# Slienteagle-wyb/tdmpc

Hardware: AMD Instinct MI355X
Metric: plan-steps/sec (N=512, H=5, iters=6) at 1/2/4/8 MI355X vs CPU ref (higher is better)
Workload: dtype fp32

## Files before the change

tdmpc_amd/csrc/tdmpc_kernels.hip:

```cpp
#include <hip/hip_runtime.h>
#include <hiprand/hiprand_kernel.h>

#include <math.h>
#include <stdint.h>
#include <stdio.h>
#include <stdlib.h>
#include <string.h>
#include <unistd.h>

#include <algorithm>
#include <atomic>
#include <chrono>
#include <mutex>
#include <type_traits>
#include <vector>

#include "../../include/tdmpc_hip.h"

typedef float floatx16 __attribute__((ext_vector_type(16)));

#define DEVI __device__ __forceinline__

#ifdef TDMPC_STAMPS
__device__ unsigned long long* g_stamps;
// ... 164 lines not shown
        w->fold_w = take((size_t)2 * w->M * w->M);
        int r, k;
        x6_shape(*w, X6_WP1, &r, &k);
        w->fpi_x6 = take(rup(r, 32) * rup(k, 16) * 3 / 2);
        w->fpi_b = take((size_t)w->M);
        x6_shape(*w, X6_WQ1X, &r, &k);
        w->fq_x6 = take(rup(r, 32) * rup(k, 16) * 3 / 2);
        w->fq_b = take((size_t)2 * w->M);
        w->fold_p = take((size_t)w->M * w->M);
        w->fold_q = take((size_t)2 * w->M * w->M);
        x6_shape(*w, X6_W1X, &r, &k);
        w->fw1_x6 = take(rup(r, 32) * rup(k, 16) * 3 / 2);
    }
    w->total = o;
    return true;
}

constexpr int SPLIT_S = 4;
constexpr int SPLIT_MAX_ROWS = 4096;

struct Work {
    float* X;
    float* H1;
    float* H2;
    float2* st1;
    float2* st2;
    float* rpart;
    float* G;
    float* rlast;
    float* value;
    float* qv;
    float* z0c;
    float* pimu;
    float* zpart;
    float* rpart_s;
    int split_rows;
    float* z0;
    float* mean;
    float* stdv;
    float* enc_tmp;
    size_t x_stride;
    int xrows;
    char* p1;
    size_t p1_bytes;
    size_t total;
};

size_t pixel_act_floats(const Layout& w) {
    size_t m = 0;
    for (int i = 1; i <= 4; ++i) m = std::max(m, (size_t)w.nch * w.conv_hw[i] * w.conv_hw[i]);
    return m;
}

constexpr int P1_NG = 8;
constexpr int P1_WPG = 32;
constexpr int P1_RTM = 3;
constexpr int P1_ROWS = 32 * P1_RTM;
constexpr int P1_H1LD = 544;
constexpr unsigned P1_XCC_TAB = P1_NG * 256 + 256;
constexpr unsigned P1_SPIN_MAX = 400000;

struct P1Region {
    unsigned o_sync, o_xb, o_h1, o_zp, o_rp, o_pp, o_qm, o_qp, o_val, o_rl, o_mu, o_y2, xb_t, xb_g, total;
};

inline int p1_ks(const Layout& w) { return (w.Kx + 31) / 32 <= 4 ? 4 : 6; }
// ... 31 lines not shown
    const size_t HA = (size_t)H * A;
    return ((size_t)32 * 3 * 64 * 4 + (size_t)P1_ROWS * 36 + 2 * P1_ROWS + p1_cem_floats(H, K, A, T) +
            3 * rup(HA, 4) + 64 + 64 + 16 + 32 + 648) * 4;
}

inline bool p1_dims_ok(const tdmpc_dims* d, const Layout& w) {
    if (w.M != 512 || d->num_elites > 64) return false;
    const int N = d->num_samples, P = d->num_pi, T = N + P;
    const int sr = (N + P1_NG - 1) / P1_NG, pr = (P + P1_NG - 1) / P1_NG;
    if (sr + pr > P1_ROWS || T > 1024) return false;
    if ((w.Kx + 15) / 16 > 12 || (w.Lp + 15) / 16 > 12 || w.Lr > 128 || w.Ar > 128) return false;
    return p1_lds_bytes(d->max_horizon, d->num_elites, w.A, T) <= 160 * 1024;
}

void make_work(const tdmpc_dims* d, const Layout& w, char* base, Work* k, int extra = 0) {
    const size_t B = d->max_batch, N = d->num_samples, P = d->num_pi, T = N + P + extra, H = d->max_horizon;
    const size_t M = w.M;
    size_t o = 0;
    auto take = [&](size_t bytes) { size_t r = o; o += rup(bytes, 256); return base ? base + r : nullptr; };
    k->xrows = (int)rup(B * T, 32);
    k->x_stride = (size_t)k->xrows * w.Kx;
    k->X = (float*)take((H + 1) * k->x_stride * 4);
    k->H1 = (float*)take((size_t)k->xrows * 2 * M * 4);
    k->H2 = (float*)take((size_t)k->xrows * 2 * M * 4);
    k->st1 = (float2*)take(B * T * (2 * M / 64) * 8);
    k->st2 = (float2*)take(B * T * (2 * M / 64) * 8);
    k->rpart = (float*)take(B * T * (M / 32) * 4);
    k->G = (float*)take(B * T * 4);
    k->rlast = (float*)take(B * T * 4);
    k->value = (float*)take(B * T * 4);
    k->qv = (float*)take(2 * (size_t)k->xrows * 4);
    k->pimu = (float*)take((size_t)k->xrows * w.Ap * 4);
    k->z0c = (float*)take(B * 2 * M * 4);
    k->split_rows = std::min(k->xrows, SPLIT_MAX_ROWS);
    k->zpart = (float*)take((size_t)2 * SPLIT_S * k->split_rows * std::max(w.Lr, w.Ar) * 4);
    k->rpart_s = (float*)take((size_t)2 * SPLIT_S * k->split_rows * 4);
    k->z0 = (float*)take(B * w.Lp * 4);
    k->mean = (float*)take(B * H * w.A * 4);
    k->stdv = (float*)take(B * H * w.A * 4);
    k->enc_tmp = (float*)take(d->modality ? 2 * B * pixel_act_floats(w) * 4 : 256);
    k->p1_bytes = p1_dims_ok(d, w) && !extra ? p1_region(d, w).total : 0;
    k->p1 = k->p1_bytes ? (char*)take(k->p1_bytes) : nullptr;
    k->total = o;
}

size_t cem_lds_bytes(int T, int H, int K, int A) {
    const size_t nl = (T + 63) / 64;
    return nl * 64 * 8 + ((size_t)H * K * A + 64 + 4 * rup((size_t)H * A, 4) + 64 + 32) * 4;
}

bool check_dims(const tdmpc_dims* d) {
    if (!d) return false;
    if (d->num_samples <= 0 || d->num_pi < 0 || d->num_elites <= 0 || d->max_horizon <= 0 ||
        d->max_horizon > 16 || d->max_iterations <= 0 || d->max_batch <= 0) return false;
    const int T = d->num_samples + d->num_pi;
    if (d->num_elites > T || d->num_elites > 64 || T > 4096) return false;
    Layout w;
    if (!make_layout(d, &w)) return false;
    if (w.Kx > 1024 || w.M > 1024 || w.L > 1024 || w.A > 256 || w.E > 1024) return false;
    if (cem_lds_bytes(T, d->max_horizon, d->num_elites, w.A) > 160 * 1024) return false;
    return true;
}

DEVI float elu1(float x) { return x > 0.f ? x : expm1f(x); }
DEVI float fmul(float a, float b) { return __fmul_rn(a, b); }
DEVI float fadd(float a, float b) { return __fadd_rn(a, b); }
// ... 2514 lines not shown
    X(1, 1, 1, 1, 1, 32, false) X(1, 1, 1, 1, 1, 64, false) X(1, 1, 1, 1, 1, 128, false)              \
    X(1, 2, 1, 1, 1, 32, false) X(1, 2, 1, 1, 1, 64, false) X(1, 2, 1, 1, 1, 128, false)              \
    X(2, 2, 2, 2, 1, 1, true)

#define LDS_FOR_EACH(X) X(2, 1, 2, 4, 32) X(3, 1, 2, 4, 32) X(1, 1, 2, 2, 32)
#define CHAIN_FOR_EACH(X)                                                                            \
    X(CH_STEP, 1, 8, 4, 8, 0) X(CH_STEP, 2, 8, 4, 8, 0) X(CH_STEP, 4, 8, 4, 8, 0)                     \
    X(CH_PI, 1, 8, 4, 8, 0) X(CH_PI, 2, 8, 4, 8, 0) X(CH_PI, 4, 8, 4, 8, 0)                           \
    X(CH_Q, 1, 8, 4, 8, 0) X(CH_Q, 2, 8, 4, 8, 0) X(CH_Q, 4, 8, 4, 8, 0)                              \
    X(CH_STEP, 2, 8, 2, X6_D3, 1) X(CH_STEP, 4, 4, 2, 2, 1) X(CH_PI, 2, 8, 2, X6_D3, 1)               \
    X(CH_PI, 4, 4, 2, 2, 1) X(CH_Q, 2, 8, 2, X6_D3, 1) X(CH_Q, 4, 4, 2, 2, 1)
#define CHAIN16_FOR_EACH(X)                                                                          \
    X(CH_STEP, 2, 4, 4, 0) X(CH_STEP, 4, 4, 4, 0) X(CH_PI, 2, 4, 4, 0) X(CH_PI, 4, 4, 4, 0)           \
    X(CH_Q, 2, 4, 4, 0) X(CH_Q, 4, 4, 4, 0)                                                           \
    X(CH_STEP, 4, 4, 4, 1) X(CH_PI, 4, 4, 4, 1) X(CH_Q, 4, 4, 4, 1)
#define SPLIT_FOR_EACH(X) X(4, 4, 1) X(4, 4, 0)
#define CONV_TILE_FOR_EACH(X) X(1) X(2) X(4)
#define PLAN1_FOR_EACH(X) X(4) X(6)

int init_attrs() {
    static int done = 0;
    if (done) return 0;
    int rc = 0;
#define LINEAR_ATTR(...) rc |= set_max_lds<linear_kernel<__VA_ARGS__>>();
    FOR_EACH_LINEAR(LINEAR_ATTR)
#undef LINEAR_ATTR
    rc |= set_max_lds<cem_kernel>();
#define PLAN1_ATTR(KS) rc |= set_max_lds<plan1_kernel<KS>>();
    PLAN1_FOR_EACH(PLAN1_ATTR)
#undef PLAN1_ATTR
#define WIDE_ATTR(...) rc |= set_max_lds<wide_step_kernel<__VA_ARGS__>>();
    WIDE_FOR_EACH(WIDE_ATTR)
#undef WIDE_ATTR
#define WIDE_HEADS_ATTR(...) rc |= set_max_lds<wide_heads_kernel<__VA_ARGS__>>();
    WIDE_HEADS_FOR_EACH(WIDE_HEADS_ATTR)
#undef WIDE_HEADS_ATTR
    rc |= set_max_lds<qstat_chol_kernel>();
#define CONV_ATTR(PX) rc |= set_max_lds<conv_tile_kernel<PX>>();
    CONV_TILE_FOR_EACH(CONV_ATTR)
#undef CONV_ATTR
#define LDS_ATTR(...) rc |= set_max_lds<linear_lds_kernel<__VA_ARGS__, true>>() | set_max_lds<linear_lds_kernel<__VA_ARGS__, false>>();
    LDS_FOR_EACH(LDS_ATTR)
#undef LDS_ATTR
#define CHAIN_ATTR(...) rc |= set_max_lds<chain_kernel<__VA_ARGS__>>();
    CHAIN_FOR_EACH(CHAIN_ATTR)
#undef CHAIN_ATTR
#define CHAIN16_ATTR(...) rc |= set_max_lds<chain16_kernel<__VA_ARGS__>>();
    CHAIN16_FOR_EACH(CHAIN16_ATTR)
#undef CHAIN16_ATTR
    if (rc) return TDMPC_E_HIP;
    done = 1;
    return 0;
}

struct Profiler {
    int armed = 0, cfg = 0, pro = -1, n = 0, cap = 0, kdim = 0, rows = 0;
    hipEvent_t* ev = nullptr;
    double flops = 0.0;
    char kernel[128] = "";
};
thread_local Profiler g_prof;

bool prof_armed() { return g_prof.armed && g_prof.n + 2 <= g_prof.cap; }
hipError_t prof_begin(bool on, hipStream_t s) { return on ? hipEventRecord(g_prof.ev[g_prof.n], s) : hipSuccess; }
hipError_t prof_end(bool on, hipStream_t s, double flops) {
    if (!on) return hipSuccess;
    Profiler& pf = g_prof;
// ... 705 lines not shown
            p.X1 = (const unsigned short*)(c.pw + w.fq_x6) + q * x6_w1_rows_stride(c);
            p.b1 = c.pw + w.fq_b + q * M;
        }
    }
    a.q = qo ? qo : c.k.qv; a.q_ld = qo ? q_ld : c.k.xrows;
    return launch_chain(CH_Q, a, 2, c.s);
}

int wh_g1p(const Ctx& c) { return (int)rup(c.w.Lp, 32) / 32; }
int wh_nb3p(const Ctx& c) { return (int)rup(c.w.A, 16) / 16; }
int wh_g1q(const Ctx& c) { return (int)rup(c.Kx, 32) / 32; }
bool wh_instance(const Ctx& c) {
    const int g1p = wh_g1p(c), nb3 = wh_nb3p(c), g1q = wh_g1q(c), nst = c.w.nsr / 16;
#define WH_HAS(G1P, NB3P, G1Q, NSTQ) if (g1p == G1P && nb3 == NB3P && g1q == G1Q && nst == NSTQ) return true;
    WIDE_HEADS_FOR_EACH(WH_HAS)
#undef WH_HAS
    return false;
}
bool use_wide_heads(const Ctx& c) {
    static const int en = [] { const char* e = getenv("TDMPC_WIDE_HEADS"); return e ? atoi(e) : 1; }();
    if (!en || !c.w.nqs || c.w.M != 512 || !use_x6(c) || !num_cus()) return false;
    if (c.path != TDMPC_PATH_AUTO && c.path != TDMPC_PATH_CHAIN && c.path != TDMPC_PATH_WIDE) return false;
    if (c.N + c.P != c.T || c.N % 16 || c.P % 16) return false;
    if (!use_wide(c, c.B * c.N, RowMap{c.N, c.T, 0}, false) || !wh_instance(c)) return false;
    return c.P == 0 || use_chain(c, c.B * c.P, 1, CK_PI);
}
WHJob wh_job(int role, int head, int x0, int nx, int rows, RowMap map) {
    WHJob j;
    memset(&j, 0, sizeof j);
    j.role = role; j.head = head; j.x0 = x0; j.nx = nx; j.rows = rows; j.nrb = (rows + 127) / 128; j.map = map;
    j.eps_G = 1;
    return j;
}
int launch_wide_heads(const Ctx& c, const WHJob* jobs, int nj, const float* eps, float min_std) {
    const Layout& w = c.w;
    const int M = c.M;
    WHArgs a;
    memset(&a, 0, sizeof a);
    for (int i = 0; i < nj; ++i) a.job[i] = jobs[i];
    a.njob = nj;
    a.X = Xt(c, c.H); a.x_ts = (long)c.Kx * 32;
    auto q6 = [&](int i) { return (const unsigned short*)(c.pw + w.x6q[i]); };
    a.P1 = q6(X6_WP1); a.P2 = q6(X6_WP2); a.P3 = q6(X6_WP3);
    a.pb1 = c.pw + w.bp1; a.pb2 = c.pw + w.bp2; a.pb3 = c.pw + w.bp3;
    a.A = w.A; a.Ap = w.Ap; a.pq1 = w.Ap / 4; a.pkq = w.Lp / 4; a.pg1s = wh_g1p(c);
    a.eps = eps; a.min_std = min_std; a.lo = (float)(-1.0 + 1e-6); a.hi = (float)(1.0 - 1e-6);
    const int g1q = wh_g1q(c);
    for (int h = 0; h < 2; ++h) {
        WHQHead& q = a.q[h];
        q.S = (const unsigned short*)(c.pw + w.x6qs) + (size_t)h * (w.nsr / 16) * g1q * 1536;
        q.X1 = (const unsigned short*)(c.pw + w.x6qf) + (size_t)h * (M / 16) * g1q * 1536;
        q.X2 = q6(X6_WQ2) + (size_t)h * (M / 16) * (M / 32) * 1536;
        q.bs = c.pw + w.bqs + (size_t)h * w.nsr;
        q.b1 = c.pw + w.bqf + h * M; q.g1 = c.pw + w.g1 + h * M; q.be1 = c.pw + w.be1 + h * M;
        q.b2 = c.pw + w.bq2 + h * M; q.g2 = c.pw + w.g2 + h * M; q.be2 = c.pw + w.be2 + h * M;
        q.w3 = c.pw + w.wq3 + h * M; q.b3 = c.pw + w.bq3 + h;
    }
    a.qkq = c.Kx / 4; a.qg1s = g1q;
    a.qv = c.k.qv; a.q_ld = c.k.xrows;
    int slots = 0;
    bool allq = true;
    double flops = 0.0;
    for (int i = 0; i < nj; ++i) {
        const WHJob& J = jobs[i];
        if (J.rows % 16 || J.x0 < 0 || J.nx <= 0 || J.x0 + J.nx > 8) {
            snprintf(g_err, sizeof g_err, "wide heads: bad job %d", i);
            return TDMPC_E_DIMS;
        }
        slots = std::max(slots, (J.nrb + J.nx - 1) / J.nx);
        allq = allq && J.role == WH_Q;
        flops += 2.0 * J.rows * (J.role == WH_PI ? (double)w.L * M + (double)M * M + (double)M * w.A
                                                 : (double)(w.L + w.A) * M + (double)M * M + M);
    }
    if (!slots) return 0;
    const dim3 grid((unsigned)slots * 8), block(64 * WS_NW);
    const int g1p = wh_g1p(c), nb3 = wh_nb3p(c), nst = w.nsr / 16;
    Profiler& pf = g_prof;
    const bool prof = prof_armed() && pf.cfg == 4 + (allq ? CH_Q : CH_PI) && (pf.rows == 0 || jobs[0].rows == pf.rows);
    if (prof)
        snprintf(pf.kernel, sizeof pf.kernel, "wide_heads_kernel<%d, %d, %d, %d> (%s)", g1p, nb3, g1q, nst,
                 allq ? "Q1 + Q2" : "pi + Q1 + Q2 of the policy rows");
    HIPCHK(prof_begin(prof, c.s));
    bool done = false;
#define WH_LAUNCH(G1P, NB3P, G1Q, NSTQ) \
    if (!done && g1p == G1P && nb3 == NB3P && g1q == G1Q && nst == NSTQ) { \
        hipLaunchKernelGGL((wide_heads_kernel<G1P, NB3P, G1Q, NSTQ>), grid, block, \
                           ws_lds<(G1P > G1Q ? G1P : G1Q)>(), c.s, a); \
        done = true; \
    }
    WIDE_HEADS_FOR_EACH(WH_LAUNCH)
#undef WH_LAUNCH
    if (!done) { snprintf(g_err, sizeof g_err, "wide heads: no instance"); return TDMPC_E_DIMS; }
    HIPCHK(hipGetLastError());
    HIPCHK(prof_end(prof, c.s, flops));
    return 0;
}

int terminal_wide(const Ctx& c, const float* noise, long toff, float min_std) {
    const RowMap rm = {c.N, c.T, 0}, pm = {c.P, c.T, c.N};
    WHJob ja[3];
    int na = 0;
    ja[na] = wh_job(WH_PI, 0, 0, c.P > 0 ? 4 : 8, c.B * c.N, rm);
    ja[na].eps_env = c.eps_env; ja[na].eps_off = toff; ja[na].eps_G = c.N;
    ++na;
    if (c.P > 0) {
        ja[na++] = wh_job(WH_Q, 0, 4, 2, c.B * c.P, pm);
        ja[na++] = wh_job(WH_Q, 1, 6, 2, c.B * c.P, pm);
    }
    int rc;
    if ((rc = launch_wide_heads(c, ja, na, noise, min_std))) return rc;
    const WHJob jb[2] = {wh_job(WH_Q, 0, 0, 4, c.B * c.N, rm), wh_job(WH_Q, 1, 4, 4, c.B * c.N, rm)};
    return launch_wide_heads(c, jb, 2, noise, min_std);
}

int terminal_q_rows(const Ctx& c, int rows, RowMap map, float discH, bool chain) {
    const Layout& w = c.w;
    const int M = c.M;
    int rc;
    if (chain) return q_chain(c, rows, map);
    {
        LinArgs a = args0();
        a.M = rows; a.K = c.Kx; a.a_mapped = 1; a.amap = map;
        LinProb& p = a.p[0];
        p.A = xop(c, c.H, 0); p.W = wop(c, w.wq1x, c.Kx); p.bias = c.pw + w.bq1x;
        p.C = hout(c.k.H1, c, 0); p.N = p.nvalid = p.nstore = 2 * M; p.epi = EPI_LNSTATS;
        p.st_out = c.k.st1; p.st_ld = 2 * M / 64;
        if ((rc = launch_lin(a, 1, 2 * M, 1, PRO_PLAIN, c.s))) return rc;
    }
    {
        LnArgs l;
        l.Y = c.k.H1; l.O = c.k.H2; l.ts = (long)2 * M * 32; l.st = c.k.st1; l.st_ld = 2 * M / 64; l.M_ = M;
        l.rows = rows; l.g = c.pw + w.g1; l.b = c.pw + w.be1;
        hipLaunchKernelGGL(ln_tanh_kernel, dim3((rows + 31) / 32, 2), dim3(512), 0, c.s, l);
        HIPCHK(hipGetLastError());
    }
    {
        LinArgs a = args0();
        a.M = rows; a.K = M;
        for (int q = 0; q < 2; ++q) {
            LinProb& p = a.p[q];
            p.A = hop(c.k.H2, c, q * M / 4); p.W = wop(c, w.wq2 + (size_t)q * M * M, M);
            p.bias = c.pw + w.bq2 + q * M; p.C = hout(c.k.H1, c, q * M / 4); p.N = p.nvalid = p.nstore = M;
            p.epi = EPI_LNSTATS; p.st_out = c.k.st2 + q * (M / 64); p.st_ld = 2 * M / 64;
// ... 467 lines not shown
        }
    }

    const RowMap all = {T, T, 0};
    const RowMap pm = {P, T, N};
    const RowMap rm = {N, T, 0};
    if (P > 0) {
        for (int t = 0; t < H; ++t) {
            if ((rc = policy(c, t, B * P, pm, noise, c.eps_env, P, (long)t * P * c.A, prm->min_std, nullptr,
                             c.fold_policy && t >= 1)))
                return rc;
            if ((rc = step_next(c, t, B * T, all, prm->discount_pow[t], t == 0, t == H - 1)))
                return rc;
        }
    }
    CemArgs ca = cem_args0(c);
    ca.I = I;
    ca.eps = noise; ca.eps_env = c.eps_env; ca.eps_cem_off = c.eps_cem_off; ca.eps_iter = c.eps_iter;
    ca.eps_act_off = c.eps_act_off; ca.u = u; ca.prev_mean = prev_mean;
    ca.eval_mode = prm->eval_mode; ca.temperature = prm->temperature; ca.momentum = prm->momentum;
    ca.omm = prm->one_minus_momentum; ca.std_floor = prm->std_floor; ca.action = action; ca.metrics = metrics;
    ca.std_floor_p = prm->std_floor_dev;
    ca.elite_out = elite_out; ca.score_out = score_out; ca.mean_out = mean_out; ca.std_out = std_out;
    ca.value_out = value_out;
    ca.status = prm->status;
    const bool wide_heads = use_wide_heads(c);
    if (wide_heads || c.fold_heads || use_chain(c, B * T, 2, CK_Q)) {
        ca.G = c.k.G; ca.qv = c.k.qv; ca.q_ld = c.k.xrows; ca.discH = prm->discount_pow[H];
    }
    const size_t cem_lds = cem_lds_bytes(T, H, ca.K, c.A);

    const bool pi_cache = pi_cache_on() && P > 0 && use_chain(c, B * T, 1, CK_PI);
    const RowMap pmH = {P, T, N};
    for (int i = 0; i < I; ++i) {
        const long toff = c.eps_cem_off + (long)i * c.eps_iter + c.eps_term_off;
        const bool pm_in_prep = wide_heads && P > 0 && i > 0;
        if (i > 0) {
            const PiMuArgs pm = pimu_args(c, B * P, pmH, noise, c.eps_env, P, toff + (long)N * c.A, prm->min_std);
            if ((rc = prep(c, noise, i, nullptr, pm_in_prep ? &pm : nullptr))) return rc;
        }
        if (i > 0 || P == 0)
            for (int t = 0; t < H; ++t)
                if ((rc = step_next(c, t, B * N, rm, prm->discount_pow[t], t == 0, t == H - 1, 1)))
                    return rc;
        if (wide_heads) {
            if (P > 0) {
                if (i == 0) rc = policy(c, H, B * P, pmH, noise, c.eps_env, P, toff + (long)N * c.A, prm->min_std, c.k.pimu);
                if (rc || (rc = flush_split(c))) return rc;
            }
            if ((rc = terminal_wide(c, noise, toff, prm->min_std))) return rc;
        } else if (c.fold_heads) {
            if ((rc = policy(c, H, B * N, rm, noise, c.eps_env, N, toff, prm->min_std, nullptr, true))) return rc;
            if (P > 0) {
                if (i == 0 || !pi_cache)
                    rc = policy(c, H, B * P, pmH, noise, c.eps_env, P, toff + (long)N * c.A, prm->min_std,
                                pi_cache ? c.k.pimu : nullptr, c.fold_policy != 0);
                else
                    rc = policy_from_mu(c, B * P, pmH, noise, c.eps_env, P, toff + (long)N * c.A, prm->min_std);
                if (rc) return rc;
            }
            if ((rc = q_chain(c, B * N, rm, nullptr, nullptr, 0, true))) return rc;
            if (P > 0 && (rc = q_chain(c, B * P, pmH, nullptr, nullptr, 0, c.fold_policy != 0))) return rc;
        } else if (pi_cache && i > 0) {
            if ((rc = policy(c, H, B * N, rm, noise, c.eps_env, N, toff, prm->min_std))) return rc;
            if ((rc = flush_split(c))) return rc;
            if ((rc = policy_from_mu(c, B * P, pmH, noise, c.eps_env, P, toff + (long)N * c.A, prm->min_std)))
                return rc;
        } else if ((rc = policy(c, H, B * T, all, noise, c.eps_env, T, toff, prm->min_std,
                                pi_cache ? c.k.pimu : nullptr))) {
            return rc;
        }
        if (!wide_heads && !c.fold_heads && (rc = terminal_q(c, prm->discount_pow[H]))) return rc;
        ca.final_iter = i == I - 1;
        ca.iter = i;
        hipLaunchKernelGGL(cem_kernel, dim3(B), dim3(1024), cem_lds, c.s, ca);
        HIPCHK(hipGetLastError());
    }
    return 0;
}

int tdmpc_icem_sizes_for(const tdmpc_dims* d, tdmpc_sizes* out) {
    if (!d || !out) return TDMPC_E_NULL;
    if (!check_dims(d)) return TDMPC_E_DIMS;
// ... 225 lines not shown
```

tdmpc_amd/csrc/wide_heads.inc:

```

enum { WH_PI = 0, WH_Q = 1 };

#if (defined(WH_DIAG_ELU) || defined(WH_DIAG_NOSTATS) || defined(WH_DIAG_NOLN2)) && !defined(TDMPC_VARIANT)
#error "WH_DIAG_* diagnostics produce wrong results: build them only as a named variant (tdmpc_amd.build --variant)"
#endif
#ifdef WH_DIAG_NOSTATS
constexpr int WH_STATS_ON = 0;
#else
constexpr int WH_STATS_ON = 1;
#endif

struct WHJob {
    int role, head;
    int x0, nx;
    int rows, nrb;
    RowMap map;
    long eps_env, eps_off;
    int eps_G;
};

struct WHQHead {
    const unsigned short* S;
    const unsigned short* X1;
    const unsigned short* X2;
    const float* bs;
    const float *b1, *g1, *be1, *b2, *g2, *be2, *w3, *b3;
};

struct WHArgs {
    WHJob job[3]; int njob;
    float* X; long x_ts;
    const unsigned short *P1, *P2, *P3;
    const float *pb1, *pb2, *pb3;
    int A, Ap, pq1, pkq, pg1s;
    const float* eps; float min_std, lo, hi;
    WHQHead q[2];
    int qkq, qg1s;
    float* qv; long q_ld;
};

template <int G> constexpr size_t wh_lds() { return ws_lds<G>(); }

DEVI float wh_u(float x) { return __builtin_bit_cast(float, __builtin_amdgcn_readfirstlane(__builtin_bit_cast(int, x))); }
DEVI const w2cf* wh_cp(const float* p) {
    const unsigned long long u = (unsigned long long)p;
    const unsigned lo = __builtin_amdgcn_readfirstlane((unsigned)u), hi = __builtin_amdgcn_readfirstlane((unsigned)(u >> 32));
    return (const w2cf*)(((unsigned long long)hi << 32) | lo);
}

template <int G1, int NB3, int GX>
DEVI void wh_pi(const WHArgs& a, const WHJob& J, int rb, char* wsm) {
    constexpr int NS = ws_ns<GX>();
    constexpr int VM = 3 * (NS - 3);
    constexpr int SPC2 = G1 + 16;
    static_assert(NS >= 3 && NS - 1 < SPC2, "ring depth");
    const int tid = threadIdx.x, lane = tid & 63, n = lane & 15, q = lane >> 4;
    const int wave = __builtin_amdgcn_readfirstlane(tid >> 6);
    char* ring = wsm;
    p1f4* sx = (p1f4*)(wsm + NS * WS_SLOT) + wave * (G1 * 2 * 64) + lane;
    const float* sb2 = (const float*)(wsm + NS * WS_SLOT);
    const float* sb3 = sb2 + 512;
    const int m0 = rb * 128 + wave * 16;
    const bool live = m0 < J.rows;
    const int xr0 = live ? map_row(J.map, m0) : 0;
    const unsigned ring_lds = (unsigned)(size_t)(__attribute__((address_space(3))) char*)ring;
    const unsigned voff = lane * 16;
    auto src_main2 = [&](int sc, int j) __attribute__((always_inline)) -> const unsigned short* {
        if (j < G1) return a.P1 + ((size_t)(8 * sc + wave) * a.pg1s + j) * 1536;
        const int s2 = j - G1, co = s2 >> 3, st = s2 & 7;
        return a.P2 + ((size_t)(8 * (st & 3) + wave) * 16 + 2 * (2 * sc + co) + (st >> 2)) * 1536;
    };
// ... 144 lines not shown
        }
    }
    asm volatile("s_waitcnt vmcnt(0)" ::: "memory");
    if (live) {
        const int m = m0 + n_ep, xr = xr0 + n_ep;
        const float* ep = a.eps + (size_t)(m / J.eps_G) * J.eps_env + J.eps_off + (size_t)(m % J.eps_G) * a.A;
        float* xo = a.X + (size_t)(xr >> 5) * a.x_ts + (xr & 31) * 4;
#pragma unroll
        for (int jj = 0; jj < NB3; ++jj) {
            const int cq = 4 * jj + q_ep, col = 4 * cq;
            if (col < a.Ap) {
                const float4 bv = *(const float4*)(sb3 + col);
                const float o4[4] = {a3[jj][0] + bv.x, a3[jj][1] + bv.y, a3[jj][2] + bv.z, a3[jj][3] + bv.w};
                float o[4];
#pragma unroll
                for (int e = 0; e < 4; ++e) {
                    float x = 0.f;
                    if (col + e < a.A) {
                        const float muv = tanhf(o4[e]);
                        x = muv;
                        if (a.min_std > 0.f) {
                            const float ee = tclamp(fmul(ep[col + e], a.min_std), -0.3f, 0.3f);
                            x = tclamp(fadd(muv, ee), a.lo, a.hi);
                        }
                    }
                    o[e] = x;
                }
                *(float4*)(xo + (size_t)cq * 128) = make_float4(o[0], o[1], o[2], o[3]);
            }
        }
    }
}

template <int G1, int NST, int GX>
DEVI void wh_q(const WHArgs& a, const WHJob& J, int rb, char* wsm) {
    constexpr int NS = ws_ns<GX>();
    constexpr int VM = 3 * (NS - 3);
    constexpr int SPC2 = G1 + 16;
    constexpr int NSS = WH_STATS_ON * (NST / 8) * G1;
    static_assert(NST % 8 == 0 && NS >= 3 && NS - 1 < SPC2 && NS - 1 <= NSS + SPC2, "ring depth");
    const int tid = threadIdx.x, lane = tid & 63, n = lane & 15, q = lane >> 4;
    const int wave = __builtin_amdgcn_readfirstlane(tid >> 6);
    const WHQHead Hd = J.head ? a.q[1] : a.q[0];
    char* ring = wsm;
    p1f4* sx = (p1f4*)(wsm + NS * WS_SLOT) + wave * (G1 * 2 * 64) + lane;
    const float* sv = (const float*)(wsm + NS * WS_SLOT);
    const int m0 = rb * 128 + wave * 16;
    const bool live = m0 < J.rows;
    const int xr0 = live ? map_row(J.map, m0) : 0;
    const unsigned ring_lds = (unsigned)(size_t)(__attribute__((address_space(3))) char*)ring;
    const unsigned voff = lane * 16;
    auto src_main2 = [&](int sc, int j) __attribute__((always_inline)) -> const unsigned short* {
        if (sc > 3) return Hd.X2;
        if (j < G1) return Hd.X1 + ((size_t)(8 * sc + wave) * a.qg1s + j) * 1536;
        const int s2 = j - G1, co = s2 >> 3, st = s2 & 7;
        return Hd.X2 + ((size_t)(8 * (st & 3) + wave) * 16 + 2 * (2 * sc + co) + (st >> 2)) * 1536;
    };
    auto src_abs = [&](int j) __attribute__((always_inline)) -> const unsigned short* {
        if (j < NSS) return Hd.S + ((size_t)(8 * (j / G1) + wave) * a.qg1s + j % G1) * 1536;
        return src_main2((j - NSS) / SPC2, (j - NSS) % SPC2);
    };
    auto src_next2 = [&](int sc, int j) __attribute__((always_inline)) -> const unsigned short* {
        const int jt = j + NS - 1;
        if (jt < SPC2) return src_main2(sc, jt);
        return src_main2(sc + 1, jt - SPC2);
    };
    auto issue = [&](int k, const unsigned short* src) __attribute__((always_inline)) {
        const unsigned dst = ring_lds + (unsigned)((k % NS) * WS_SLOT + wave * WS_FRAG);
#pragma unroll
        for (int p = 0; p < 3; ++p) w2_glds(src + p * 512, voff, dst + p * 1024);
    };
#pragma unroll
    for (int k = 0; k < NS - 1; ++k) issue(k, src_abs(k));
    const float* xp = a.X + (size_t)(xr0 >> 5) * a.x_ts + ((xr0 & 31) + n) * 4;
    const p1f4 zero4 = {0.f, 0.f, 0.f, 0.f};
    float xsum = 0.f;
#pragma unroll
    for (int g = 0; g < G1; ++g) {
        const int qa = 8 * g + q, qb = qa + 4;
        const p1f4 va = live && qa < a.qkq ? *(const p1f4*)(xp + (size_t)qa * 128) : zero4;
        const p1f4 vb = live && qb < a.qkq ? *(const p1f4*)(xp + (size_t)qb * 128) : zero4;
        sx[(2 * g) * 64] = va;
        sx[(2 * g + 1) * 64] = vb;
        xsum += ((va[0] + va[1]) + (va[2] + va[3])) + ((vb[0] + vb[1]) + (vb[2] + vb[3]));
    }
    const bool xfin = ws_wave_finite(xsum);
    asm volatile("s_waitcnt vmcnt(0) lgkmcnt(0)\n\ts_barrier" ::: "memory");

    int k = 0;
    auto sync = [&](const unsigned short* nsrc, bool tail_bias = false) __attribute__((always_inline)) -> const char* {
        asm volatile("s_waitcnt vmcnt(%0)\n\ts_barrier" :: "n"(VM) : "memory");
        const char* sl = ring + (k % NS) * WS_SLOT + lane * 16;
        issue(k + NS - 1, nsrc);
        if (tail_bias) {
            const float* vs[4] = {Hd.b2, Hd.g2, Hd.be2, Hd.w3};
            w2_glds(vs[wave >> 1] + 256 * (wave & 1), voff, ring_lds + (unsigned)(NS * WS_SLOT) + wave * 1024);
        }
        ++k;
        return sl;
    };
    uint4 fc[WS_AHEAD][3];
    auto rd = [&](uint4 (&f)[3], const char* p) __attribute__((always_inline)) {
        f[0] = *(const uint4*)p;
        f[1] = *(const uint4*)(p + 1024);
        f[2] = *(const uint4*)(p + 2048);
    };
#pragma unroll
    for (int d = 0; d < WS_AHEAD; ++d) rd(fc[d], ring + d * WS_FRAG + lane * 16);
    auto frag = [&](const char* sl, int i, uint4& w0, uint4& w1, uint4& w2) __attribute__((always_inline)) {
        w0 = fc[0][0];
        w1 = fc[0][1];
        w2 = fc[0][2];
#pragma unroll
        for (int d = 0; d + 1 < WS_AHEAD; ++d)
#pragma unroll
            for (int p = 0; p < 3; ++p) fc[d][p] = fc[d + 1][p];
        rd(fc[WS_AHEAD - 1], i + WS_AHEAD <= WS_NW - 1 ? sl + (i + WS_AHEAD) * WS_FRAG
                                                       : ring + (k % NS) * WS_SLOT + (i + WS_AHEAD - WS_NW) * WS_FRAG + lane * 16);
        __builtin_amdgcn_sched_barrier(0);
    };
    const bool qb0 = (q & 1) != 0, qb1 = (q & 2) != 0;
    const w2cf* vb1 = wh_cp(Hd.b1);
    const w2cf* vbe1 = wh_cp(Hd.be1);
    const w2cf* vbs = wh_cp(Hd.bs);
    auto vec4 = [&](const w2cf* v, int t, int i) __attribute__((always_inline)) -> float {
        const w2cf* p = v + 16 * t;
        const float c0 = wh_u(p[i]), c1 = wh_u(p[4 + i]), c2 = wh_u(p[8 + i]), c3 = wh_u(p[12 + i]);
        const float lo = qb0 ? c1 : c0, hi = qb0 ? c3 : c2;
        return qb1 ? hi : lo;
    };

    float mean_l = 0.f, ssq = 0.f;
#pragma unroll
    for (int ss = 0; ss < WH_STATS_ON * NST / 8; ++ss) {
        floatx4 as[8];
#pragma unroll
        for (int b = 0; b < 8; ++b) as[b] = floatx4{0.f, 0.f, 0.f, 0.f};
#pragma unroll
        for (int g = 0; g < G1; ++g) {
            const char* sl = sync(src_abs(ss * G1 + g + NS - 1));
            const p1f4 x0 = sx[(2 * g) * 64], x1 = sx[(2 * g + 1) * 64];
            const WSX xb = ws_opnd(make_float4(x0[0], x0[1], x0[2], x0[3]), make_float4(x1[0], x1[1], x1[2], x1[3]), xfin);
#pragma unroll
            for (int b = 0; b < 8; ++b) {
                uint4 w0, w1, w2;
                frag(sl, b, w0, w1, w2);
                ws_prod(as[b], w0, w1, w2, xb);
            }
        }
#pragma unroll
        for (int b = 0; b < 8; ++b)
#pragma unroll
            for (int i = 0; i < 4; ++i) {
                const float s = as[b][i] + vec4(vbs, 8 * ss + b, i);
                if (ss == 0 && b == 0 && i == 0) mean_l = s;
                else ssq += s * s;
            }
    }
    if (q != 0) ssq += mean_l * mean_l;
    ssq += __shfl_xor(ssq, 16);
    ssq += __shfl_xor(ssq, 32);
    const float rs1 = 1.0f / sqrtf(ssq / 512.f + 1e-5f);
    (void)mean_l;

    floatx4 acc[32];
#pragma unroll
    for (int j = 0; j < 32; ++j) acc[j] = floatx4{0.f, 0.f, 0.f, 0.f};
#pragma unroll 1
    for (int sc = 0; sc < 4; ++sc) {
        floatx4 a1[8];
#pragma unroll
        for (int b = 0; b < 8; ++b) a1[b] = floatx4{0.f, 0.f, 0.f, 0.f};
#pragma unroll
        for (int g = 0; g < G1; ++g) {
            const char* sl = sync(src_next2(sc, g));
            const p1f4 x0 = sx[(2 * g) * 64], x1 = sx[(2 * g + 1) * 64];
            const WSX xb = ws_opnd(make_float4(x0[0], x0[1], x0[2], x0[3]), make_float4(x1[0], x1[1], x1[2], x1[3]), xfin);
#pragma unroll
            for (int b = 0; b < 8; ++b) {
                uint4 w0, w1, w2;
                frag(sl, b, w0, w1, w2);
                ws_prod(a1[b], w0, w1, w2, xb);
            }
        }
#pragma unroll
        for (int co = 0; co < 2; ++co) {
            const int c = 2 * sc + co;
#pragma unroll
            for (int b = 0; b < 4; ++b)
#pragma unroll
                for (int i = 0; i < 4; ++i) {
                    const float v = a1[4 * co + b][i] + vec4(vb1, 4 * c + b, i);
#ifndef WH_DIAG_ELU
                    a1[4 * co + b][i] = tanh_f(fadd(fmul(v, rs1), vec4(vbe1, 4 * c + b, i)));
#else
                    a1[4 * co + b][i] = elu_f(v);
#endif
                }
            const floatx4* t = a1 + 4 * co;
            const bool hfin = ws_wave_finite(ws_sum8(make_float4(t[0][0], t[0][1], t[0][2], t[0][3]),
                                                     make_float4(t[1][0], t[1][1], t[1][2], t[1][3])) +
                                             ws_sum8(make_float4(t[2][0], t[2][1], t[2][2], t[2][3]),
                                                     make_float4(t[3][0], t[3][1], t[3][2], t[3][3])));
#pragma unroll
            for (int s2 = 0; s2 < 2; ++s2) {
                const floatx4& t0 = t[2 * s2];
                const floatx4& t1 = t[2 * s2 + 1];
                const WSX xb = ws_opnd(make_float4(t0[0], t0[1], t0[2], t0[3]), make_float4(t1[0], t1[1], t1[2], t1[3]), hfin);
#pragma unroll
                for (int jq = 0; jq < 4; ++jq) {
                    const char* sl = sync(src_next2(sc, G1 + 8 * co + 4 * s2 + jq), sc == 3 && co == 0 && s2 == 0 && jq == 0);
#pragma unroll
                    for (int jj = 0; jj < 8; ++jj) {
                        uint4 w0, w1, w2;
                        frag(sl, jj, w0, w1, w2);
                        ws_prod(acc[8 * jq + jj], w0, w1, w2, xb);
                    }
                }
            }
        }
    }
    asm volatile("s_waitcnt vmcnt(0)\n\ts_barrier" ::: "memory");
    int l16 = (int)voff;
    asm volatile("" : "+v"(l16));
    const int n_ep = (l16 >> 4) & 15, q_ep = (l16 >> 8) & 3;
    auto lv = [&](int vsel, int t) __attribute__((always_inline)) -> float4 {
        return *(const float4*)(sv + vsel * 512 + 16 * t + 4 * q_ep);
    };
#ifdef WH_DIAG_NOLN2
    if (live && q_ep == 0) a.qv[(size_t)J.head * a.q_ld + xr0 + n_ep] = acc[0][0] + acc[31][3] + rs1;
    return;
#endif
    float s = 0.f;
#pragma unroll
    for (int t = 0; t < 32; ++t) {
        const float4 bv = lv(0, t);
        acc[t][0] += bv.x; acc[t][1] += bv.y; acc[t][2] += bv.z; acc[t][3] += bv.w;
#pragma unroll
        for (int i = 0; i < 4; ++i) s += acc[t][i];
    }
    s += __shfl_xor(s, 16);
    s += __shfl_xor(s, 32);
    const float mean2 = s / 512.f;
    float v2 = 0.f;
#pragma unroll
    for (int t = 0; t < 32; ++t)
#pragma unroll
        for (int i = 0; i < 4; ++i) {
            const float d = acc[t][i] - mean2;
            v2 += d * d;
        }
    v2 += __shfl_xor(v2, 16);
    v2 += __shfl_xor(v2, 32);
    const float rs2 = 1.0f / sqrtf(v2 / 512.f + 1e-5f);
    const float sh2 = -rs2 * mean2;
    float o = 0.f;
#pragma unroll
    for (int t = 0; t < 32; ++t) {
        const float4 gv = lv(1, t), bv = lv(2, t), wv = lv(3, t);
        const float gg[4] = {gv.x, gv.y, gv.z, gv.w}, bb[4] = {bv.x, bv.y, bv.z, bv.w};
        float y[4];
#pragma unroll
        for (int i = 0; i < 4; ++i) y[i] = elu_f(fadd(fmul(fadd(fmul(acc[t][i], rs2), sh2), gg[i]), bb[i]));
        o += (y[0] * wv.x + y[1] * wv.y) + (y[2] * wv.z + y[3] * wv.w);
    }
    o += __shfl_xor(o, 16);
    o += __shfl_xor(o, 32);
    if (live && q_ep == 0) a.qv[(size_t)J.head * a.q_ld + xr0 + n_ep] = o + Hd.b3[0];
}

template <int G1P, int NB3P, int G1Q, int NSTQ>
__global__ void __launch_bounds__(64 * WS_NW) __attribute__((amdgpu_waves_per_eu(2, 2)))
wide_heads_kernel(const WHArgs a) {
    constexpr int GX = G1P > G1Q ? G1P : G1Q;
    extern __shared__ __attribute__((aligned(16))) char wsm[];
    const int bid = blockIdx.x, xg = bid & 7, slot = bid >> 3;
    int j = -1;
#pragma unroll
    for (int i = 0; i < 3; ++i)
        if (i < a.njob && xg >= a.job[i].x0 && xg < a.job[i].x0 + a.job[i].nx) j = i;
    if (j < 0) return;
    const WHJob J = j == 0 ? a.job[0] : j == 1 ? a.job[1] : a.job[2];
    const int rb = slot * J.nx + (xg - J.x0);
    if (rb >= J.nrb) return;
    if (J.role == WH_PI) wh_pi<G1P, NB3P, GX>(a, J, rb, wsm);
    else wh_q<G1Q, NSTQ, GX>(a, J, rb, wsm);
}

#define WIDE_HEADS_FOR_EACH(X) X(4, 2, 4, 8) X(4, 3, 5, 16) X(2, 1, 2, 8) X(2, 1, 3, 8)

__host__ __device__ inline int qs_col(int i, int A, int L, int Ap) { return i < A ? i : i < A + L ? Ap + (i - A) : -1; }
__host__ __device__ inline size_t qs_pidx(int r, int k, int pk) {
    return ((size_t)(r >> 5) * (pk / 4) + (k >> 2)) * 128 + (r & 31) * 4 + (k & 3);
}

struct QStatArgs {
    const float* W1;
    const float* b1;
    double* gram;
    int M, Kx, A, L, Ap, n;
    unsigned short* S;
    float* bs;
    int nsr, g1s;
    unsigned short* F;
    float* bf;
    const float* g1;
};

DEVI float qs_val(const QStatArgs& a, int h, int m, int i) {
    const int k = qs_col(i, a.A, a.L, a.Ap);
    return k >= 0 ? a.W1[qs_pidx(h * a.M + m, k, a.Kx)] : a.b1[h * a.M + m];
}

DEVI void qs_means(const QStatArgs& a, int h, int c0, double* mu, double* part) {
    const int tid = threadIdx.x, col = tid & 31, p = tid >> 5;
    double s = 0.0;
    if (c0 + col < a.n)
        for (int m = p; m < a.M; m += 8) s += (double)qs_val(a, h, m, c0 + col);
    part[p * 32 + col] = s;
// ... 107 lines not shown
```

Baseline: 6321.

## Cache latent-only Q first-layer partials for policy rows across CEM iterations

```diff
diff --git a/tdmpc_amd/csrc/tdmpc_kernels.hip b/tdmpc_amd/csrc/tdmpc_kernels.hip
--- a/tdmpc_amd/csrc/tdmpc_kernels.hip
+++ b/tdmpc_amd/csrc/tdmpc_kernels.hip
@@ -220,6 +220,8 @@
     float* qv;
     float* z0c;
     float* pimu;
+    float* qsh;
+    size_t qsh_head;
     float* zpart;
     float* rpart_s;
     int split_rows;
@@ -317,6 +319,8 @@
     k->qv = (float*)take(2 * (size_t)k->xrows * 4);
     k->pimu = (float*)take((size_t)k->xrows * w.Ap * 4);
     k->z0c = (float*)take(B * 2 * M * 4);
+    k->qsh_head = M == 512 && w.nqs && P > 0 && P % 16 == 0 ? (B * P + 127) / 128 * 8 * (32 + w.nsr / 16) * 256 : 0;
+    k->qsh = (float*)take(k->qsh_head ? 2 * k->qsh_head * 4 : 256);
     k->split_rows = std::min(k->xrows, SPLIT_MAX_ROWS);
     k->zpart = (float*)take((size_t)2 * SPLIT_S * k->split_rows * std::max(w.Lr, w.Ar) * 4);
     k->rpart_s = (float*)take((size_t)2 * SPLIT_S * k->split_rows * 4);
@@ -2897,7 +2901,8 @@
 #define WIDE_ATTR(...) rc |= set_max_lds<wide_step_kernel<__VA_ARGS__>>();
     WIDE_FOR_EACH(WIDE_ATTR)
 #undef WIDE_ATTR
-#define WIDE_HEADS_ATTR(...) rc |= set_max_lds<wide_heads_kernel<__VA_ARGS__>>();
+#define WIDE_HEADS_ATTR(...) rc |= set_max_lds<wide_heads_kernel<__VA_ARGS__, 0>>(); \
+    rc |= set_max_lds<wide_heads_kernel<__VA_ARGS__, 1>>(); rc |= set_max_lds<wide_heads_kernel<__VA_ARGS__, 2>>();
     WIDE_HEADS_FOR_EACH(WIDE_HEADS_ATTR)
 #undef WIDE_HEADS_ATTR
     rc |= set_max_lds<qstat_chol_kernel>();
@@ -3669,7 +3674,7 @@
     j.eps_G = 1;
     return j;
 }
-int launch_wide_heads(const Ctx& c, const WHJob* jobs, int nj, const float* eps, float min_std) {
+int launch_wide_heads(const Ctx& c, const WHJob* jobs, int nj, const float* eps, float min_std, int sh = 0) {
     const Layout& w = c.w;
     const int M = c.M;
     WHArgs a;
@@ -3695,6 +3700,7 @@
     }
     a.qkq = c.Kx / 4; a.qg1s = g1q;
     a.qv = c.k.qv; a.q_ld = c.k.xrows;
+    a.qsh = c.k.qsh;
     int slots = 0;
     bool allq = true;
     double flops = 0.0;
@@ -3704,6 +3710,11 @@
             snprintf(g_err, sizeof g_err, "wide heads: bad job %d", i);
             return TDMPC_E_DIMS;
         }
+        if (sh && J.role == WH_Q && (!c.k.qsh_head || J.sh_off != (long)(J.head * c.k.qsh_head) ||
+                                     (size_t)J.nrb * 8 * (32 + w.nsr / 16) * 256 > c.k.qsh_head)) {
+            snprintf(g_err, sizeof g_err, "wide heads: share job %d outside the cache", i);
+            return TDMPC_E_DIMS;
+        }
         slots = std::max(slots, (J.nrb + J.nx - 1) / J.nx);
         allq = allq && J.role == WH_Q;
         flops += 2.0 * J.rows * (J.role == WH_PI ? (double)w.L * M + (double)M * M + (double)M * w.A
@@ -3715,14 +3726,16 @@
     Profiler& pf = g_prof;
     const bool prof = prof_armed() && pf.cfg == 4 + (allq ? CH_Q : CH_PI) && (pf.rows == 0 || jobs[0].rows == pf.rows);
     if (prof)
-        snprintf(pf.kernel, sizeof pf.kernel, "wide_heads_kernel<%d, %d, %d, %d> (%s)", g1p, nb3, g1q, nst,
+        snprintf(pf.kernel, sizeof pf.kernel, "wide_heads_kernel<%d, %d, %d, %d, %d> (%s)", g1p, nb3, g1q, nst, sh,
                  allq ? "Q1 + Q2" : "pi + Q1 + Q2 of the policy rows");
     HIPCHK(prof_begin(prof, c.s));
     bool done = false;
 #define WH_LAUNCH(G1P, NB3P, G1Q, NSTQ) \
     if (!done && g1p == G1P && nb3 == NB3P && g1q == G1Q && nst == NSTQ) { \
-        hipLaunchKernelGGL((wide_heads_kernel<G1P, NB3P, G1Q, NSTQ>), grid, block, \
-                           ws_lds<(G1P > G1Q ? G1P : G1Q)>(), c.s, a); \
+        const size_t lds = ws_lds<(G1P > G1Q ? G1P : G1Q)>(); \
+        if (sh == 0) hipLaunchKernelGGL((wide_heads_kernel<G1P, NB3P, G1Q, NSTQ, 0>), grid, block, lds, c.s, a); \
+        else if (sh == 1) hipLaunchKernelGGL((wide_heads_kernel<G1P, NB3P, G1Q, NSTQ, 1>), grid, block, lds, c.s, a); \
+        else hipLaunchKernelGGL((wide_heads_kernel<G1P, NB3P, G1Q, NSTQ, 2>), grid, block, lds, c.s, a); \
         done = true; \
     }
     WIDE_HEADS_FOR_EACH(WH_LAUNCH)
@@ -3733,7 +3746,11 @@
     return 0;
 }
 
-int terminal_wide(const Ctx& c, const float* noise, long toff, float min_std) {
+bool q_share_on() {
+    const char* e = getenv("TDMPC_Q_SHARE");
+    return !e || atoi(e) != 0;
+}
+int terminal_wide(const Ctx& c, const float* noise, long toff, float min_std, int sh) {
     const RowMap rm = {c.N, c.T, 0}, pm = {c.P, c.T, c.N};
     WHJob ja[3];
     int na = 0;
@@ -3743,9 +3760,12 @@
     if (c.P > 0) {
         ja[na++] = wh_job(WH_Q, 0, 4, 2, c.B * c.P, pm);
         ja[na++] = wh_job(WH_Q, 1, 6, 2, c.B * c.P, pm);
+        ja[na - 1].sh_off = (long)c.k.qsh_head;
+    } else {
+        sh = 0;
     }
     int rc;
-    if ((rc = launch_wide_heads(c, ja, na, noise, min_std))) return rc;
+    if ((rc = launch_wide_heads(c, ja, na, noise, min_std, sh))) return rc;
     const WHJob jb[2] = {wh_job(WH_Q, 0, 0, 4, c.B * c.N, rm), wh_job(WH_Q, 1, 4, 4, c.B * c.N, rm)};
     return launch_wide_heads(c, jb, 2, noise, min_std);
 }
@@ -4279,6 +4299,7 @@
 
     const bool pi_cache = pi_cache_on() && P > 0 && use_chain(c, B * T, 1, CK_PI);
     const RowMap pmH = {P, T, N};
+    const bool q_share = wide_heads && P > 0 && I > 1 && q_share_on();
     for (int i = 0; i < I; ++i) {
         const long toff = c.eps_cem_off + (long)i * c.eps_iter + c.eps_term_off;
         const bool pm_in_prep = wide_heads && P > 0 && i > 0;
@@ -4295,7 +4316,8 @@
                 if (i == 0) rc = policy(c, H, B * P, pmH, noise, c.eps_env, P, toff + (long)N * c.A, prm->min_std, c.k.pimu);
                 if (rc || (rc = flush_split(c))) return rc;
             }
-            if ((rc = terminal_wide(c, noise, toff, prm->min_std))) return rc;
+            if ((rc = terminal_wide(c, noise, toff, prm->min_std, q_share ? (i == 0 ? 1 : 2) : 0)))
+                return rc;
         } else if (c.fold_heads) {
             if ((rc = policy(c, H, B * N, rm, noise, c.eps_env, N, toff, prm->min_std, nullptr, true))) return rc;
             if (P > 0) {
diff --git a/tdmpc_amd/csrc/wide_heads.inc b/tdmpc_amd/csrc/wide_heads.inc
--- a/tdmpc_amd/csrc/wide_heads.inc
+++ b/tdmpc_amd/csrc/wide_heads.inc
@@ -17,6 +17,7 @@
     RowMap map;
     long eps_env, eps_off;
     int eps_G;
+    long sh_off;
 };
 
 struct WHQHead {
@@ -37,6 +38,7 @@
     WHQHead q[2];
     int qkq, qg1s;
     float* qv; long q_ld;
+    float* qsh;
 };
 
 template <int G> constexpr size_t wh_lds() { return ws_lds<G>(); }
@@ -247,13 +249,20 @@
     }
 }
 
-template <int G1, int NST, int GX>
+template <int G1, int NST, int GX, int SH, int NB3>
 DEVI void wh_q(const WHArgs& a, const WHJob& J, int rb, char* wsm) {
     constexpr int NS = ws_ns<GX>();
     constexpr int VM = 3 * (NS - 3);
-    constexpr int SPC2 = G1 + 16;
-    constexpr int NSS = WH_STATS_ON * (NST / 8) * G1;
+    constexpr int GA = SH ? (NB3 + 1) / 2 : 0;
+    constexpr int TA = SH ? NB3 + 1 : 0;
+    constexpr int L1F = SH == 2 ? 0 : G1;
+    constexpr int L1A = SH == 2 ? GA : 0;
+    constexpr int SPC2 = L1F + L1A + 16;
+    constexpr int NSF = SH == 2 ? 0 : WH_STATS_ON * (NST / 8) * G1;
+    constexpr int NSS = NSF + (SH == 2 ? WH_STATS_ON : 0);
+    constexpr int CT = (32 + NST) * 256;
     static_assert(NST % 8 == 0 && NS >= 3 && NS - 1 < SPC2 && NS - 1 <= NSS + SPC2, "ring depth");
+    static_assert(TA * GA <= WS_NW && GA <= G1 && TA <= NST, "the action step");
     const int tid = threadIdx.x, lane = tid & 63, n = lane & 15, q = lane >> 4;
     const int wave = __builtin_amdgcn_readfirstlane(tid >> 6);
     const WHQHead Hd = J.head ? a.q[1] : a.q[0];
@@ -267,12 +276,17 @@
     const unsigned voff = lane * 16;
     auto src_main2 = [&](int sc, int j) __attribute__((always_inline)) -> const unsigned short* {
         if (sc > 3) return Hd.X2;
-        if (j < G1) return Hd.X1 + ((size_t)(8 * sc + wave) * a.qg1s + j) * 1536;
-        const int s2 = j - G1, co = s2 >> 3, st = s2 & 7;
+        if (j < L1F) return Hd.X1 + ((size_t)(8 * sc + wave) * a.qg1s + j) * 1536;
+        if (j < L1F + L1A) return Hd.X1 + ((size_t)(8 * sc + wave) * a.qg1s + (j - L1F)) * 1536;
+        const int s2 = j - L1F - L1A, co = s2 >> 3, st = s2 & 7;
         return Hd.X2 + ((size_t)(8 * (st & 3) + wave) * 16 + 2 * (2 * sc + co) + (st >> 2)) * 1536;
     };
     auto src_abs = [&](int j) __attribute__((always_inline)) -> const unsigned short* {
-        if (j < NSS) return Hd.S + ((size_t)(8 * (j / G1) + wave) * a.qg1s + j % G1) * 1536;
+        if (j < NSF) return Hd.S + ((size_t)(8 * (j / G1) + wave) * a.qg1s + j % G1) * 1536;
+        if (j < NSS) {
+            const int f = SH && wave < TA * GA ? wave : 0;
+            return Hd.S + ((size_t)(f / (GA ? GA : 1)) * a.qg1s + f % (GA ? GA : 1)) * 1536;
+        }
         return src_main2((j - NSS) / SPC2, (j - NSS) % SPC2);
     };
     auto src_next2 = [&](int sc, int j) __attribute__((always_inline)) -> const unsigned short* {
@@ -289,18 +303,34 @@
     for (int k = 0; k < NS - 1; ++k) issue(k, src_abs(k));
     const float* xp = a.X + (size_t)(xr0 >> 5) * a.x_ts + ((xr0 & 31) + n) * 4;
     const p1f4 zero4 = {0.f, 0.f, 0.f, 0.f};
+    const int apq = a.Ap / 4, xq = SH == 2 ? apq : a.qkq;
     float xsum = 0.f;
 #pragma unroll
-    for (int g = 0; g < G1; ++g) {
+    for (int g = 0; g < (SH == 2 ? GA : G1); ++g) {
         const int qa = 8 * g + q, qb = qa + 4;
-        const p1f4 va = live && qa < a.qkq ? *(const p1f4*)(xp + (size_t)qa * 128) : zero4;
-        const p1f4 vb = live && qb < a.qkq ? *(const p1f4*)(xp + (size_t)qb * 128) : zero4;
+        const p1f4 va = live && qa < xq ? *(const p1f4*)(xp + (size_t)qa * 128) : zero4;
+        const p1f4 vb = live && qb < xq ? *(const p1f4*)(xp + (size_t)qb * 128) : zero4;
         sx[(2 * g) * 64] = va;
         sx[(2 * g + 1) * 64] = vb;
         xsum += ((va[0] + va[1]) + (va[2] + va[3])) + ((vb[0] + vb[1]) + (vb[2] + vb[3]));
     }
     const bool xfin = ws_wave_finite(xsum);
+    float* const cp = SH ? a.qsh + J.sh_off + (size_t)(rb * WS_NW + wave) * CT + lane * 4 : nullptr;
+    floatx4 asl[SH ? NST : 1];
+    if constexpr (SH == 2) {
+#pragma unroll
+        for (int t = 0; t < NST; ++t) asl[t] = *(const floatx4*)(cp + (32 + t) * 256);
+    }
     asm volatile("s_waitcnt vmcnt(0) lgkmcnt(0)\n\ts_barrier" ::: "memory");
+    auto xpart = [&](int g, int part) __attribute__((always_inline)) -> WSX {
+        p1f4 x0 = sx[(2 * g) * 64], x1 = sx[(2 * g + 1) * 64];
+        if (part) {
+            const bool k0 = (8 * g + q < apq) == (part == 2), k1 = (8 * g + 4 + q < apq) == (part == 2);
+            x0 = k0 ? x0 : zero4;
+            x1 = k1 ? x1 : zero4;
+        }
+        return ws_opnd(make_float4(x0[0], x0[1], x0[2], x0[3]), make_float4(x1[0], x1[1], x1[2], x1[3]), xfin);
+    };
 
     int k = 0;
     auto sync = [&](const unsigned short* nsrc, bool tail_bias = false) __attribute__((always_inline)) -> const char* {
@@ -346,31 +376,63 @@
     };
 
     float mean_l = 0.f, ssq = 0.f;
-#pragma unroll
-    for (int ss = 0; ss < WH_STATS_ON * NST / 8; ++ss) {
+    auto stat = [&](int t, int i, float s) __attribute__((always_inline)) {
+        if (t == 0 && i == 0) mean_l = s;
+        else ssq += s * s;
+    };
+    floatx4 asa[SH ? TA : 1];
+#pragma unroll
+    for (int t = 0; t < (SH ? TA : 1); ++t) asa[t] = floatx4{0.f, 0.f, 0.f, 0.f};
+#pragma unroll
+    for (int ss = 0; ss < NSF / G1; ++ss) {
         floatx4 as[8];
 #pragma unroll
         for (int b = 0; b < 8; ++b) as[b] = floatx4{0.f, 0.f, 0.f, 0.f};
 #pragma unroll
         for (int g = 0; g < G1; ++g) {
             const char* sl = sync(src_abs(ss * G1 + g + NS - 1));
-            const p1f4 x0 = sx[(2 * g) * 64], x1 = sx[(2 * g + 1) * 64];
-            const WSX xb = ws_opnd(make_float4(x0[0], x0[1], x0[2], x0[3]), make_float4(x1[0], x1[1], x1[2], x1[3]), xfin);
+            const WSX xb = xpart(g, SH ? 1 : 0);
+            WSX xa = xb;
+            if constexpr (SH == 1)
+                if (g < GA) xa = xpart(g, 2);
 #pragma unroll
             for (int b = 0; b < 8; ++b) {
                 uint4 w0, w1, w2;
                 frag(sl, b, w0, w1, w2);
                 ws_prod(as[b], w0, w1, w2, xb);
-            }
-        }
-#pragma unroll
-        for (int b = 0; b < 8; ++b)
-#pragma unroll
-            for (int i = 0; i < 4; ++i) {
-                const float s = as[b][i] + vec4(vbs, 8 * ss + b, i);
-                if (ss == 0 && b == 0 && i == 0) mean_l = s;
-                else ssq += s * s;
-            }
+                if constexpr (SH == 1)
+                    if (g < GA && 8 * ss + b < TA) ws_prod(asa[8 * ss + b < TA ? 8 * ss + b : 0], w0, w1, w2, xa);
+            }
+        }
+#pragma unroll
+        for (int b = 0; b < 8; ++b) {
+            if constexpr (SH) {
+                asl[8 * ss + b] = as[b];
+                *(floatx4*)(cp + (32 + 8 * ss + b) * 256) = as[b];
+            } else {
+#pragma unroll
+                for (int i = 0; i < 4; ++i) stat(8 * ss + b, i, as[b][i] + vec4(vbs, 8 * ss + b, i));
+            }
+        }
+    }
+    if constexpr (SH == 2 && WH_STATS_ON) {
+        WSX xa[GA];
+#pragma unroll
+        for (int g = 0; g < GA; ++g) xa[g] = xpart(g, 0);
+        const char* sl = sync(src_abs(NSF + NS - 1));
+#pragma unroll
+        for (int f = 0; f < WS_NW; ++f) {
+            uint4 w0, w1, w2;
+            frag(sl, f, w0, w1, w2);
+            if (f < TA * GA) ws_prod(asa[f / GA], w0, w1, w2, xa[f % GA]);
+        }
+    }
+    if constexpr (SH != 0 && WH_STATS_ON) {
+#pragma unroll
+        for (int t = 0; t < NST; ++t)
+#pragma unroll
+            for (int i = 0; i < 4; ++i)
+                stat(t, i, ((t < TA ? asa[t < TA ? t : 0][i] : 0.f) + asl[t][i]) + vec4(vbs, t, i));
     }
     if (q != 0) ssq += mean_l * mean_l;
     ssq += __shfl_xor(ssq, 16);
@@ -386,17 +448,49 @@
         floatx4 a1[8];
 #pragma unroll
         for (int b = 0; b < 8; ++b) a1[b] = floatx4{0.f, 0.f, 0.f, 0.f};
-#pragma unroll
-        for (int g = 0; g < G1; ++g) {
+        floatx4 e1[SH ? 8 : 1];
+        if constexpr (SH == 2) {
+#pragma unroll
+            for (int b = 0; b < 8; ++b) e1[b] = *(const floatx4*)(cp + (8 * sc + b) * 256);
+        }
+        if constexpr (SH == 1) {
+#pragma unroll
+            for (int b = 0; b < 8; ++b) e1[b] = floatx4{0.f, 0.f, 0.f, 0.f};
+        }
+#pragma unroll
+        for (int g = 0; g < L1F; ++g) {
             const char* sl = sync(src_next2(sc, g));
-            const p1f4 x0 = sx[(2 * g) * 64], x1 = sx[(2 * g + 1) * 64];
-            const WSX xb = ws_opnd(make_float4(x0[0], x0[1], x0[2], x0[3]), make_float4(x1[0], x1[1], x1[2], x1[3]), xfin);
+            const WSX xb = xpart(g, SH ? 1 : 0);
+            WSX xa = xb;
+            if constexpr (SH == 1)
+                if (g < GA) xa = xpart(g, 2);
 #pragma unroll
             for (int b = 0; b < 8; ++b) {
                 uint4 w0, w1, w2;
                 frag(sl, b, w0, w1, w2);
                 ws_prod(a1[b], w0, w1, w2, xb);
-            }
+                if constexpr (SH == 1)
+                    if (g < GA) ws_prod(e1[b], w0, w1, w2, xa);
+            }
+        }
+        if constexpr (SH == 1) {
+#pragma unroll
+            for (int b = 0; b < 8; ++b) *(floatx4*)(cp + (8 * sc + b) * 256) = a1[b];
+        }
+#pragma unroll
+        for (int g = 0; g < L1A; ++g) {
+            const char* sl = sync(src_next2(sc, L1F + g));
+            const WSX xb = xpart(g, 0);
+#pragma unroll
+            for (int b = 0; b < 8; ++b) {
+                uint4 w0, w1, w2;
+                frag(sl, b, w0, w1, w2);
+                ws_prod(a1[b], w0, w1, w2, xb);
+            }
+        }
+        if constexpr (SH != 0) {
+#pragma unroll
+            for (int b = 0; b < 8; ++b) a1[b] += e1[b];
         }
 #pragma unroll
         for (int co = 0; co < 2; ++co) {
@@ -424,7 +518,7 @@
                 const WSX xb = ws_opnd(make_float4(t0[0], t0[1], t0[2], t0[3]), make_float4(t1[0], t1[1], t1[2], t1[3]), hfin);
 #pragma unroll
                 for (int jq = 0; jq < 4; ++jq) {
-                    const char* sl = sync(src_next2(sc, G1 + 8 * co + 4 * s2 + jq), sc == 3 && co == 0 && s2 == 0 && jq == 0);
+                    const char* sl = sync(src_next2(sc, L1F + L1A + 8 * co + 4 * s2 + jq), sc == 3 && co == 0 && s2 == 0 && jq == 0);
 #pragma unroll
                     for (int jj = 0; jj < 8; ++jj) {
                         uint4 w0, w1, w2;
@@ -484,7 +578,7 @@
     if (live && q_ep == 0) a.qv[(size_t)J.head * a.q_ld + xr0 + n_ep] = o + Hd.b3[0];
 }
 
-template <int G1P, int NB3P, int G1Q, int NSTQ>
+template <int G1P, int NB3P, int G1Q, int NSTQ, int SH>
 __global__ void __launch_bounds__(64 * WS_NW) __attribute__((amdgpu_waves_per_eu(2, 2)))
 wide_heads_kernel(const WHArgs a) {
     constexpr int GX = G1P > G1Q ? G1P : G1Q;
@@ -499,7 +593,7 @@
     const int rb = slot * J.nx + (xg - J.x0);
     if (rb >= J.nrb) return;
     if (J.role == WH_PI) wh_pi<G1P, NB3P, GX>(a, J, rb, wsm);
-    else wh_q<G1Q, NSTQ, GX>(a, J, rb, wsm);
+    else wh_q<G1Q, NSTQ, GX, SH, NB3P>(a, J, rb, wsm);
 }
 
 #define WIDE_HEADS_FOR_EACH(X) X(4, 2, 4, 8) X(4, 3, 5, 16) X(2, 1, 2, 8) X(2, 1, 3, 8)
```

Result: no change. 6338, median of 6 (+0.3%).
